# zju3dv/EnvGS

Hardware: AMD Instinct MI355X
Metric: train iters/s (fwd+bwd of the render hot path + Adam step, one 800x800 view per GPU per iter) + render Mpix/s (higher is better)
Workload: dtype f32

## Files before the change

envgs_amd/_lib.py:

```python
import ctypes
import os

import torch

HERE = os.path.dirname(os.path.abspath(__file__))
LIB_PATH = os.path.join(HERE, "libenvgs_hip.so")
_lib = None

c_void_p, c_int, c_uint32, c_size_t = ctypes.c_void_p, ctypes.c_int, ctypes.c_uint32, ctypes.c_size_t


class RasterCfg(ctypes.Structure):
    _fields_ = [("P", ctypes.c_int32), ("sh_degree", ctypes.c_int32), ("sh_coeffs", ctypes.c_int32),
                ("channels", ctypes.c_int32), ("width", ctypes.c_int32), ("height", ctypes.c_int32),
                ("bg_len", ctypes.c_int32), ("debug", ctypes.c_int32), ("scale_modifier", ctypes.c_float),
                ("tanfovx", ctypes.c_float), ("tanfovy", ctypes.c_float), ("feature_f16", ctypes.c_int32)]


class AdamTensor(ctypes.Structure):
    _fields_ = [("param", ctypes.c_void_p), ("grad", ctypes.c_void_p), ("exp_avg", ctypes.c_void_p), ("exp_avg_sq", ctypes.c_void_p),
                ("numel", ctypes.c_int64), ("lr", ctypes.c_float), ("step", ctypes.c_float)]


class RowsTensor(ctypes.Structure):
# ... 89 lines not shown
    "envgs_raster_sort_temp_bytes": (c_size_t, [c_uint32, ctypes.c_int32, ctypes.c_int32]),
    "envgs_raster_project": (c_int, [ctypes.POINTER(RasterCfg)] + [_P] * 15 + [_P, c_size_t, ctypes.POINTER(c_uint32), _P]),
    "envgs_raster_bin_and_render": (c_int, [ctypes.POINTER(RasterCfg), c_uint32] + [_P] * 7 + [_P, c_size_t] + [_P] * 7 + [_P]),
    "envgs_raster_render_audit": (c_int, [ctypes.POINTER(RasterCfg)] + [_P] * 11 + [ctypes.c_int32, _P, _P]),
    "envgs_raster_backward": (c_int, [ctypes.POINTER(RasterCfg), c_uint32] + [_P] * 29 + [_P]),
    "envgs_bvh_temp_bytes": (c_size_t, [ctypes.c_int32]),
    "envgs_bvh_node_floats": (c_size_t, [ctypes.c_int32]),
    "envgs_bvh_build": (c_int, [ctypes.c_int32, _P, _P, _P, _P, c_size_t, ctypes.c_int32, _P]),
    "envgs_bvh_refit": (c_int, [ctypes.c_int32, _P, _P, _P, _P, _P, c_size_t, ctypes.c_int32, _P]),
    "envgs_bvh_quality": (c_int, [ctypes.c_int32, _P, _P, _P]),
    "envgs_trace_ray_sort_temp_bytes": (c_size_t, [ctypes.c_int32]),
    "envgs_trace_ray_order": (c_int, [ctypes.c_int32, _P, _P, _P, ctypes.c_int32, _P, _P, _P, c_size_t, _P]),
    "envgs_trace_forward": (c_int, [ctypes.POINTER(TraceCfg)] + [_P] * 22 + [ctypes.POINTER(TraceLists), _P]),
    "envgs_trace_backward": (c_int, [ctypes.POINTER(TraceCfg)] + [_P] * 35 + [ctypes.POINTER(TraceLists), _P]),
    "envgs_trace_backward_join": (c_int, [_P]),
    "envgs_sh_colors_forward": (c_int, [ctypes.c_int32] * 4 + [_P] * 7 + [_P]),
    "envgs_sh_colors_backward": (c_int, [ctypes.c_int32] * 4 + [_P] * 9 + [_P]),
    "envgs_surfel_quads": (c_int, [ctypes.c_int32] + [_P] * 5 + [_P]),
    "envgs_blend_forward": (c_int, [ctypes.c_int32] * 3 + [_P] * 3 + [_P]),
    "envgs_blend_backward": (c_int, [ctypes.c_int32] * 3 + [_P] * 5 + [_P]),
    "envgs_bounce_rays_forward": (c_int, [ctypes.c_int32] + [_P] * 8 + [_P]),
    "envgs_bounce_rays_backward": (c_int, [ctypes.c_int32] + [_P] * 13 + [_P]),
    "envgs_bounce_blend_forward": (c_int, [ctypes.c_int32] + [_P] * 5 + [_P]),
    "envgs_bounce_blend_backward": (c_int, [ctypes.c_int32] + [_P] * 8 + [_P]),
    "envgs_bounce_pack_mid": (c_int, [ctypes.c_int32, _P, ctypes.c_int32, ctypes.c_int32] + [_P] * 8 + [_P]),
    "envgs_reflect_forward": (c_int, [ctypes.c_int32, ctypes.c_int32, ctypes.c_float] + [_P] * 8 + [_P]),
    "envgs_reflect_backward": (c_int, [ctypes.c_int32, ctypes.c_int32, ctypes.c_float] + [_P] * 11 + [_P]),
    "envgs_select_acc": (c_int, [ctypes.c_int32, ctypes.c_int32, ctypes.c_float, _P, _P, _P]),
    "envgs_reflect_filtered_forward": (c_int, [ctypes.c_int32, ctypes.c_int32, ctypes.c_float, ctypes.c_int32] + [_P] * 10 + [_P]),
    "envgs_reflect_filtered_backward": (c_int, [ctypes.c_int32, ctypes.c_int32, ctypes.c_float, ctypes.c_int32] + [_P] * 13 + [_P]),
# ... 95 lines not shown
```

envgs_amd/csrc/trace_api.hip:

```cpp
#include "trace_common.h"

#include <mutex>

namespace envgs {

constexpr int MAX_SEG = ENVGS_TRACE_MAX_SEG;

static int persistent_grid(int R, int per_cu = 8)
{
    int dev = 0, cus = 256;
    if (hipGetDevice(&dev) == hipSuccess) {
        int v = 0;
        if (hipDeviceGetAttribute(&v, hipDeviceAttributeMultiprocessorCount, dev) == hipSuccess && v > 0) cus = v;
    }
    const int want = (R + 63) / 64;
    const int cap = cus * per_cu;
    return want < cap ? (want > 0 ? want : 1) : cap;
}

static int stride_grid(int R, int per_block)
{
    const int want = (R + per_block - 1) / per_block;
    const int cap = 256 * 32;
    const int g = want < cap ? (want > 0 ? want : 1) : cap;
// ... 74 lines not shown
    return A;
}

static int bwd_order_classes()
{
    const int k = debug_switch(ENVGS_DBG_BALANCE) >> 8;
    return k > 0 ? k : ENVGS_BWD_ORDER_CLASSES;
}

static unsigned sparse_capacity(const envgs_trace_lists *L)
{
    return (unsigned)(L->sparse_cap > 0xFFFFFFF0ull ? 0xFFFFFFF0ull : L->sparse_cap);
}

static int forward_segment(const envgs_trace_cfg *cfg, const envgs_raster_cfg *dcfg, const envgs_trace_lists *L, const TraceArgs &S, hipStream_t st,
                           int seg_wgs, bool compact)
{
    const int rays_seg = (S.batch1 - S.batch0) * 64;
    {
        ProfScope p1(K_TRACE_COLLECT, st);
        const dim3 cg(persistent_grid(rays_seg, seg_wgs));
        const float4 *n4 = S.nodes + (size_t)(cfg->P > 1 ? cfg->P - 1 : 1) * 4;
        hipLaunchKernelGGL(collect_hits_coop, cg, dim3(256), 0, st, S, S.nodes, n4, S.srec);
    }
    ENVGS_CHECK_LAUNCH(dcfg, st);
    if (compact) {
        const int nb_seg = S.batch1 - S.batch0, nblk = (rays_seg + 255) / 256;
        unsigned *cntb = L->row_blk;
        const unsigned long long limit = (unsigned long long)L->compact_rows;
        unsigned *first_row = S.counter + ENVGS_CTR_SEG_FIRST_ROW + S.seg;
        hipLaunchKernelGGL(row_scan_blocks, dim3(1), dim3(256), 0, st, cntb + S.batch0, nb_seg, S.counter + ENVGS_CTR_ROW_CLAIM, first_row);
        hipLaunchKernelGGL(row_offsets, dim3(nblk), dim3(256), 0, st, S, cntb, L->row_off, (uint2 *)L->batch_rows, (const unsigned *)first_row, limit);
        ENVGS_CHECK_LAUNCH(dcfg, st);
    }
    {
        ProfScope p2(K_TRACE_SORT, st);
        const dim3 g(stride_grid(rays_seg, 4)), b(256);
        if (S.shp) hipLaunchKernelGGL((sort_composite_fwd<4, false, true>), g, b, 0, st, S);
        else hipLaunchKernelGGL((sort_composite_fwd<4, false, false>), g, b, 0, st, S);
        if (S.cap > 256) {
            const dim3 gl(min(stride_grid(rays_seg, 256), 512));
            if (S.cap <= 512) { if (S.shp) hipLaunchKernelGGL((sort_composite_fwd<8, true, true>), gl, b, 0, st, S); else hipLaunchKernelGGL((sort_composite_fwd<8, true, false>), gl, b, 0, st, S); }
            else { if (S.shp) hipLaunchKernelGGL((sort_composite_fwd<16, true, true>), gl, b, 0, st, S); else hipLaunchKernelGGL((sort_composite_fwd<16, true, false>), gl, b, 0, st, S); }
        }
    }
    ENVGS_CHECK_LAUNCH(dcfg, st);
    {
        ProfScope p8(K_TRACE_REGISTER, st);
        const dim3 gr(stride_grid(rays_seg, 64)), br(64 * RH_W);
// ... 63 lines not shown
    if (lists) {
        if (L->scan_temp_bytes < scan_temp_bytes(cfg->P * NCOPY)) return ENVGS_ERR_TEMP_TOO_SMALL;
        A.hits = (uint2 *)L->hit_lists; A.hit_cnt = L->hit_cnt; A.n_used = L->n_used; A.cap = L->cap;
        A.surf_cnt = L->surf_cnt; A.surf_off = L->surf_off; A.surf_acc = (unsigned long long *)L->surf_acc;
        const bool will_sort = L->ray_keys && L->ray_order && L->ray_sort_temp && !(A.exp & ENVGS_DBG_TRACE_NO_SORT);
        {
            int ib = 1;
            while ((1ll << ib) <= (long long)cfg->num_rays) ib++;
            A.wfrac = 40 - ib > 30 ? 30 : 40 - ib;
        }
        A.state = (float4 *)L->hit_state; A.entries = (unsigned long long *)L->entries; A.pairs = L->pairs; A.n_entries = L->n_entries;
        const bool compact = L->compact_rows > 0 && L->row_off && L->batch_rows && L->row_blk && L->hit_state;
        if (L->compact_rows > 0 && !compact) return ENVGS_ERR_BAD_ARG;
        A.state_plane = compact ? (size_t)L->compact_rows : (size_t)cfg->num_rays * (size_t)L->cap;
        A.colour_state = L->state_planes == 1 ? 1 : 0;
        if (compact) { A.row_off = L->row_off; A.batch_rows = (const uint2 *)L->batch_rows; A.batch_cnt = L->row_blk; }
        if (L->sparse_hits && L->sparse_cap > 0 && L->entries && L->pairs && L->hit_state) {
            const int sw = debug_switch(ENVGS_DBG_SPARSE);
            A.sparse = (uint4 *)L->sparse_hits;
            A.sparse_cap = sparse_capacity(L);
            A.sparse_max = sw > 0 ? (sw - 1 > 64 ? 64 : sw - 1) : 4;
        }
        if (L->sh_perm && shs && cfg->sh_coeffs == 16) {
            const size_t nw = (size_t)cfg->P * 48;
            FP.perm_blocks = (int)((nw + 255) / 256); FP.nb = (cfg->sh_degree + 1) * (cfg->sh_degree + 1); FP.f16 = cfg->feature_f16;
            FP.shs = (const void *)shs; FP.shp = L->sh_perm;
            A.shp = L->sh_perm;
        }
        const int nbatch_all = (cfg->num_rays + 63) / 64;
        int nseg = 2;
        if (debug_switch(ENVGS_DBG_SEGMENTS) > 0) nseg = debug_switch(ENVGS_DBG_SEGMENTS);
// ... 26 lines not shown
        }
        if (prepare_aside) { if (hipStreamWaitEvent(stream, ev_join[1], 0) != hipSuccess) return ENVGS_ERR_BAD_ARG; }
        else { const int rcp = launch_prepare(stream); if (rcp) return rcp; ENVGS_CHECK_LAUNCH(dcfg, stream); }
        if (nseg > 1) {
            if (hipEventRecord(ev_fork, stream) != hipSuccess) return ENVGS_ERR_BAD_ARG;
            for (int i = 1; i < nseg; i++)
                if (hipStreamWaitEvent(aux[i], ev_fork, 0) != hipSuccess) return ENVGS_ERR_BAD_ARG;
        }
        const int coop_wgs = (debug_switch(ENVGS_DBG_COLLECT_WGS) > 0 && debug_switch(ENVGS_DBG_COLLECT_WGS) <= 8) ? debug_switch(ENVGS_DBG_COLLECT_WGS)
                                                                                                                  : (nseg > 1 ? 4 : 8);
        for (int sg = 0; sg < nseg; sg++) {
            TraceArgs S = A;
            S.seg = sg;
            S.batch0 = (int)((long long)nbatch_all * sg / nseg);
            S.batch1 = (int)((long long)nbatch_all * (sg + 1) / nseg);
            const int rcs = forward_segment(cfg, dcfg, L, S, sg ? aux[sg] : stream, coop_wgs, compact); if (rcs) return rcs;
        }
        for (int i = 1; i < nseg; i++)
            if (hipEventRecord(ev_join[i], aux[i]) != hipSuccess || hipStreamWaitEvent(stream, ev_join[i], 0) != hipSuccess) return ENVGS_ERR_BAD_ARG;
        unsigned *bwd_order = (L->bwd_order && records_prepared(L)) ? L->bwd_order : nullptr;
        hipLaunchKernelGGL(unpack_surfel_acc, dim3((cfg->P + 255) / 256 + (bwd_order ? 1 : 0)), dim3(256), 0, stream, cfg->P, A.wfrac, A.surf_acc, L->surf_cnt, wet,
                           counters + ENVGS_CTR_RAY_FETCH, (const int *)L->n_entries, nbatch_all, bwd_order, bwd_order_classes());
        ENVGS_CHECK_LAUNCH(dcfg, stream);
        const int rc = launch_scan(L->surf_cnt, L->surf_off, cfg->P * NCOPY, L->scan_temp, L->scan_temp_bytes, stream); if (rc) return rc;
        A.only_overflow = 1;
    } else {
        const int rcp = launch_prepare(stream); if (rcp) return rcp;
        ENVGS_CHECK_LAUNCH(dcfg, stream);
    }
    { ProfScope p4(K_TRACE_KBUF_FWD, stream); hipLaunchKernelGGL(trace_fwd, dim3(persistent_grid(cfg->num_rays)), dim3(64), 0, stream, A, rh, rw); }
    ENVGS_CHECK_LAUNCH(dcfg, stream);
// ... 40 lines not shown
    if (A.exp & ENVGS_DBG_TRACE_RETIRED) return ENVGS_ERR_BAD_ARG;
    int rh, rw; ray_layout(cfg, &rh, &rw);
    bool deferred = false, have_records = false;
    int def_dev = 0;
    {
        ProfScope prof_(K_TRACE_BWD, stream);
        if (lists_wanted(cfg, L) && !lists_usable_bwd(cfg, L)) return ENVGS_ERR_BAD_ARG;
        if (lists_usable_bwd(cfg, L)) {
            A.hits = (uint2 *)L->hit_lists; A.hit_cnt = L->hit_cnt; A.n_used = L->n_used; A.cap = L->cap;
            if (L->ray_keys && L->ray_order && L->ray_sort_temp && !(A.exp & ENVGS_DBG_TRACE_NO_SORT)) A.order = L->ray_order + cfg->num_rays;
            if (L->records && L->num_records > 0 && records_prepared(L)) {
                A.surf_cnt = L->surf_cnt; A.surf_off = L->surf_off; A.records = L->records; A.num_records = L->num_records;
                A.state = (float4 *)L->hit_state; A.entries = (unsigned long long *)L->entries; A.pairs = L->pairs; A.n_entries = L->n_entries;
                if (L->compact_rows > 0) {
                    if (!L->row_off || !L->batch_rows) return ENVGS_ERR_BAD_ARG;
                    A.row_off = L->row_off; A.batch_rows = (const uint2 *)L->batch_rows;
                }
                A.state_plane = L->compact_rows > 0 ? (size_t)L->compact_rows : (size_t)cfg->num_rays * (size_t)L->cap;
                {
                    ProfScope p5(K_TRACE_LIST_BWD, stream);
                    const bool rgb_only = dL_drgb && !dL_ddpt && !dL_dacc && !dL_dnorm && !dL_daux;
                    if (L->state_planes == 1 && !rgb_only) return ENVGS_ERR_BAD_ARG;
                    const bool by_cost = L->bwd_order && !(debug_switch(ENVGS_DBG_BALANCE) & 1);
                    A.bwd_order = by_cost ? L->bwd_order : nullptr;
                    const dim3 g(by_cost ? (cfg->num_rays + 63) / 64 : stride_grid((cfg->num_rays + 63) / 64, 1));
                    if (rgb_only) hipLaunchKernelGGL((batch_surfel_bwd<true, false>), g, dim3(64), 0, stream, A);
                    else if (cfg->has_others) hipLaunchKernelGGL((batch_surfel_bwd<false, true>), g, dim3(64), 0, stream, A);
                    else hipLaunchKernelGGL((batch_surfel_bwd<false, false>), g, dim3(64), 0, stream, A);
                    if (L->sparse_hits && L->sparse_cap > 0) {
                        A.sparse = (uint4 *)L->sparse_hits;
                        A.sparse_cap = sparse_capacity(L);
// ... 47 lines not shown
```

envgs_amd/csrc/trace_collect.hip:

```cpp
#include "trace_common.h"

namespace envgs {

typedef float f32x2 __attribute__((ext_vector_type(2)));
constexpr int COOP_W = 4;
constexpr float COOP_REFRESH_OD = 1.0f;
constexpr int COOP_ODROW = 36;
constexpr int COOP_NBIN = 32;
constexpr int COOP_STK = 96;
constexpr int COOP_FRONT = 64;
constexpr int COOP_ITEMS = 256;
static_assert(COOP_ODROW % 4 == 0, "the bin rows are read with ds_read_b128");
constexpr float COOP_OD_SCALE = 65536.0f;
constexpr unsigned COOP_KILL_Q = (unsigned)(KILL_OD * 65536.0f);
struct CoopLds {
    unsigned od[64][COOP_ODROW];
    unsigned odtot[64];
    int cnt[64];
    unsigned long long items[2][COOP_ITEMS];
    int stk[COOP_W][COOP_STK];
    int nitems[2];
    int next, ovf, batch, pad;
};

__global__ void __launch_bounds__(256, 8)
collect_hits_coop(const TraceArgs A, const float4 *__restrict__ nodes, const float4 *__restrict__ nodes4, const float4 *__restrict__ srec)
{
    __shared__ CoopLds L;
#ifdef ENVGS_DIAG
// ... 60 lines not shown
            };
            const int ux = sign_of(dx, ix), uy = sign_of(dy, iy), uz = sign_of(dz, iz);
            if (vm != 0ull && ux < 2 && uy < 2 && uz < 2) oct = ux | (uy << 1) | (uz << 2);
        }
#endif

        unsigned long long c1 = c0;
        bool ovf = false;
        auto walk = [&]<int OCT>() {
        auto record_hit = [&](const SurfHit &h, const int sid) {
            const int slot = atomicAdd(&L.cnt[lane], 1);
            if (slot < A.cap) list[slot] = make_uint2(__float_as_uint(h.t), (unsigned)sid);
            const float x = (h.t - tA) * inv_bin_w;
            int b = x <= 0.0f ? 0 : (int)ceilf(x + 1e-3f);
            b = b > COOP_NBIN - 1 ? COOP_NBIN - 1 : b;
            const unsigned dep = (unsigned)(-__logf(1.0f - h.alpha) * COOP_OD_SCALE);
            atomicAdd(&L.od[lane][b], dep);
            atomicAdd(&L.odtot[lane], dep);
        };
        auto refresh_bound = [&]() {
            const unsigned tot = ENVGS_LDS_READ(L.odtot[lane]);
            if (__builtin_amdgcn_ballot_w64(tot >= COOP_KILL_Q && tot > seen + (unsigned)(COOP_REFRESH_OD * COOP_OD_SCALE)) != 0ull) {
                seen = tot;
                unsigned cum = 0u; int kb = COOP_NBIN - 1;
                const uint4 *row = reinterpret_cast<const uint4 *>(&L.od[lane][0]);
                asm volatile("" ::: "memory");
#pragma unroll
                for (int h = 0; h < COOP_NBIN / 16; h++) {
                    uint4 v[4];
#pragma unroll
                    for (int q = 0; q < 4; q++) v[q] = row[4 * h + q];
#pragma unroll
                    for (int q = 0; q < 4; q++) {
                        const unsigned e[4] = {v[q].x, v[q].y, v[q].z, v[q].w};
#pragma unroll
                        for (int j = 0; j < 4; j++) {
                            const int bin = 16 * h + 4 * q + j;
                            if (bin < COOP_NBIN - 1) { cum += e[j]; kb = (cum >= COOP_KILL_Q && kb == COOP_NBIN - 1) ? bin : kb; }
                        }
                    }
                }
                tkill = kb < COOP_NBIN - 1 ? tA + (float)kb * bin_w : tk_open;
            }
        };
        auto step = [&](const int cur_, unsigned long long (&kr)[4]) -> int {
            const int cur = __builtin_amdgcn_readfirstlane(cur_);
            const float4 *nd = nodes4 + (size_t)cur * 8;
            psteps++;
            float4 qa[4], qb[4];
#if defined(ENVGS_COOP_TIMING) && ENVGS_COOP_TIMING == 2
            const unsigned long long ta = __builtin_readcyclecounter();
            {
                typedef float f8_ __attribute__((ext_vector_type(8)));
                f8_ r0, r1, r2, r3;
                asm volatile("s_load_dwordx8 %0, %4, 0\n s_load_dwordx8 %1, %4, 32\n s_load_dwordx8 %2, %4, 64\n s_load_dwordx8 %3, %4, 96\n s_waitcnt lgkmcnt(0)"
// ... 157 lines not shown
        __syncthreads();
        const unsigned long long c3 = __builtin_readcyclecounter();
#if defined(ENVGS_COOP_TIMING) && ENVGS_COOP_TIMING == 3
        (void)c0; (void)c1; (void)c2; (void)c3;
#elif defined(ENVGS_COOP_TIMING)
        cyc_walk += c2 - c0; (void)c1; (void)c3;
#else
        cyc_expand += c1 - c0; cyc_walk += c2 - c1; cyc_wait += c3 - c2;
#endif
        if (wave == 0) {
            int n = L.cnt[lane];
            if (L.ovf) {
                n = A.cap + 1;
                if (lane == 0) atomicAdd(A.counter + ENVGS_CTR_STACK_OVERFLOWS, 1u);
            }
            if (valid) { A.hit_cnt[r] = n; found_tot += (unsigned)n; }
            int mx = n;
            for (int o = 32; o > 0; o >>= 1) mx = max(mx, __shfl_xor(mx, o));
            if (lane == 0) atomicMax((int *)(A.counter + ENVGS_CTR_MAX_LIST), mx);
            if (A.batch_cnt) {
                const float rows = wave_sum((valid && n <= A.cap) ? (float)n : 0.f);
                if (lane == 0) A.batch_cnt[A.batch0 + fb] = (unsigned)rows;
            }
        }
        __syncthreads();
    }
    if (A.stats) {
        const float ff = wave_sum((float)found_tot);
        if (lane == 0) {
            if (wave == 0) atomicAdd(A.stats + ENVGS_TOT_FOUND, (unsigned long long)ff);
            atomicAdd(A.stats + ENVGS_TOT_PACKET_NODES, (unsigned long long)psteps); atomicAdd(A.stats + ENVGS_TOT_PACKET_LEAVES, (unsigned long long)pleaves);
            atomicAdd(A.stats + ENVGS_TOT_COOP_EXPAND, cyc_expand); atomicAdd(A.stats + ENVGS_TOT_COOP_WALK, cyc_walk); atomicAdd(A.stats + ENVGS_TOT_COOP_WAIT, cyc_wait);
        }
    }
#undef ENVGS_LDS_READ
}

}
```

envgs_amd/csrc/trace_common.h:

```cpp
#ifndef ENVGS_TRACE_COMMON_H
#define ENVGS_TRACE_COMMON_H

#include "common.h"
#include "prof.h"
#include "sh_basis.h"

#include <cstdlib>
#include <cstring>

#include "../../include/envgs_trace.h"

namespace envgs {

constexpr int KBUF = 16;
constexpr int STACK = 64;
constexpr int NCOPY = 8;
constexpr int MAX_ROUNDS = 256;
constexpr float UV_MAX = 3.0f;
constexpr int MID = ENVGS_MID_CHANNELS;
constexpr int SREC = ENVGS_SREC_STRIDE;
constexpr int NODE = ENVGS_NODE_STRIDE;

struct SurfHit { float t, u, v, G, alpha, denom; bool ok; };

// ... 71 lines not shown
    int only_overflow;
    int batch0, batch1;
    uint4 *sparse;
    unsigned sparse_cap;
    int sparse_max;
    int reduce_adds;
    int seg;
    unsigned long long *entries;
    unsigned *pairs;
    int *n_entries;
    unsigned *long_list;
    float4 *state;
    size_t state_plane;
    int colour_state;
    unsigned *batch_cnt;
    const unsigned *row_off;
    const uint2 *batch_rows;
    const void *shp;
    const unsigned *bwd_order;
};

struct KBuf {
    float t[KBUF];
    int id[KBUF];
    int n;
    __device__ __forceinline__ void reset() {
#pragma unroll
        for (int i = 0; i < KBUF; i++) { t[i] = 3.0e38f; id[i] = 0x7fffffff; }
        n = 0;
    }
    __device__ __forceinline__ void insert(float ct, int cid) {
#pragma unroll
// ... 422 lines not shown
};
__global__ void __launch_bounds__(256) forward_prepare(const ForwardPrepare F);
__global__ void __launch_bounds__(64) trace_fwd(const TraceArgs A, const int ray_h, const int ray_w);
__global__ void __launch_bounds__(64) trace_bwd(const TraceArgs A, const int ray_h, const int ray_w);
__global__ void __launch_bounds__(256, 8)
collect_hits_coop(const TraceArgs A, const float4 *__restrict__ nodes, const float4 *__restrict__ nodes4, const float4 *__restrict__ srec);

template <int EMAX, bool LONG, bool QSH> __global__ void __launch_bounds__(256) sort_composite_fwd(const TraceArgs A);
extern template __global__ void __launch_bounds__(256) sort_composite_fwd<4, false, false>(const TraceArgs A);
extern template __global__ void __launch_bounds__(256) sort_composite_fwd<8, true, false>(const TraceArgs A);
extern template __global__ void __launch_bounds__(256) sort_composite_fwd<16, true, false>(const TraceArgs A);
extern template __global__ void __launch_bounds__(256) sort_composite_fwd<4, false, true>(const TraceArgs A);
extern template __global__ void __launch_bounds__(256) sort_composite_fwd<8, true, true>(const TraceArgs A);
extern template __global__ void __launch_bounds__(256) sort_composite_fwd<16, true, true>(const TraceArgs A);
template <bool CACHED> __global__ void __launch_bounds__(64 * RH_W) register_hits(const TraceArgs A);
__global__ void __launch_bounds__(256) row_scan_blocks(unsigned *__restrict__ blk, int n, unsigned *rows_used, unsigned *seg_base);
__global__ void __launch_bounds__(256) row_offsets(const TraceArgs A, const unsigned *__restrict__ blk, unsigned *__restrict__ row_off, uint2 *__restrict__ batch_rows,
                                                   const unsigned *__restrict__ seg_base, unsigned long long limit);
__global__ void __launch_bounds__(256) unpack_surfel_acc(int P, int wfrac, const unsigned long long *__restrict__ acc, unsigned *__restrict__ cnt,
                                                         float *__restrict__ wet, unsigned *ray_counter, const int *__restrict__ n_entries, int nbatch,
                                                         unsigned *__restrict__ bwd_order, int order_classes);
__global__ void __launch_bounds__(256) sparse_hits_bwd(const TraceArgs A, const int rgbo);
template <bool RGBO, bool OTH> __global__ void __attribute__((amdgpu_waves_per_eu(ENVGS_BSB_WAVES, ENVGS_BSB_WAVES))) __launch_bounds__(64) batch_surfel_bwd(const TraceArgs A);
extern template __global__ void __attribute__((amdgpu_waves_per_eu(ENVGS_BSB_WAVES, ENVGS_BSB_WAVES))) __launch_bounds__(64) batch_surfel_bwd<false, false>(const TraceArgs A);
extern template __global__ void __attribute__((amdgpu_waves_per_eu(ENVGS_BSB_WAVES, ENVGS_BSB_WAVES))) __launch_bounds__(64) batch_surfel_bwd<false, true>(const TraceArgs A);
extern template __global__ void __attribute__((amdgpu_waves_per_eu(ENVGS_BSB_WAVES, ENVGS_BSB_WAVES))) __launch_bounds__(64) batch_surfel_bwd<true, false>(const TraceArgs A);
__global__ void __launch_bounds__(256) reduce_surfel_records(const TraceArgs A);
__global__ void __launch_bounds__(256) finish_surfel_grads(int P, const float *__restrict__ rots, const float *__restrict__ geo_rec,
                                                           float *__restrict__ dmeans, float *__restrict__ dscales, float *__restrict__ dopac,
                                                           float *__restrict__ drots, float *__restrict__ dgrads3D);

}
#endif
// ... 1 lines not shown
```

envgs_amd/csrc/trace_lists.hip:

```cpp
#include "trace_common.h"

#ifndef ENVGS_SCF_KO
#define ENVGS_SCF_KO 0
#endif
namespace envgs {

template <int S>
__device__ __forceinline__ unsigned xlane(unsigned v)
{
    if constexpr (S == 1) return (unsigned)__builtin_amdgcn_update_dpp(0, (int)v, 0xB1, 0xf, 0xf, true);
    else if constexpr (S == 2) return (unsigned)__builtin_amdgcn_update_dpp(0, (int)v, 0x4E, 0xf, 0xf, true);
    else if constexpr (S == 32) {
        const envgs_u2 r = __builtin_amdgcn_permlane32_swap(v, v, false, false);
        return (threadIdx.x & 32) ? r.x : r.y;
    } else return (unsigned)__builtin_amdgcn_ds_swizzle((int)v, 0x1F | (S << 10));
}

template <int E, int SIZE, int STRIDE>
__device__ __forceinline__ void bitonic_layer(unsigned long long (&k)[E], const int lane)
{
    if constexpr (STRIDE >= 64) {
        constexpr int SE = STRIDE / 64;
#pragma unroll
        for (int e = 0; e < E; e++)
// ... 551 lines not shown
                    for (unsigned f = threadIdx.x; f < nfail; f += 64 * RH_W) {
                        const unsigned long long ev = ent[region - 1 - f];
                        const unsigned pv = prs[region - 1 - f];
                        A.sparse[fbase + f] = make_uint4((unsigned)base + (pv >> 16), pv & 0xFFFFu, (unsigned)(ev & 0xFFFFFFull), (unsigned)(ev >> 32));
                    }
                    if (threadIdx.x == 0) { if (A.n_entries) A.n_entries[2 * batch + 1] = 0; atomicSub(A.counter + ENVGS_CTR_BATCH_ENTRIES,nfail); }
                }
            }
        }
    }
}

template __global__ void register_hits<false>(const TraceArgs A);
template __global__ void register_hits<true>(const TraceArgs A);

__device__ __forceinline__ unsigned rows_of_slot(const TraceArgs &A, const int slot, const int slot_end)
{
    if (slot >= slot_end) return 0u;
    const int r = ray_of(A, slot);
    const int n = A.hit_cnt[r];
    return n > A.cap ? 0u : (unsigned)n;
}

__global__ void __launch_bounds__(256)
row_scan_blocks(unsigned *__restrict__ blk, int n, unsigned *rows_used, unsigned *seg_base)
{
    __shared__ unsigned wtot[4];
    __shared__ unsigned s_base;
    const int lane = threadIdx.x & 63, wave = threadIdx.x >> 6;
    if (threadIdx.x == 0) s_base = 0u;
    __syncthreads();
    constexpr int PRE = 8;
    unsigned pre[PRE][4];
#pragma unroll
    for (int c = 0; c < PRE; c++)
#pragma unroll
        for (int q = 0; q < 4; q++) { const int i = c * 1024 + 4 * (int)threadIdx.x + q; pre[c][q] = i < n ? blk[i] : 0u; }
    int c = 0;
    for (int c0 = 0; c0 < n; c0 += 1024, c++) {
        const int i0 = c0 + 4 * (int)threadIdx.x;
        unsigned v[4];
        if (c < PRE) {
#pragma unroll
            for (int q = 0; q < 4; q++) {
                v[q] = pre[0][q];
#pragma unroll
                for (int p_ = 1; p_ < PRE; p_++) v[q] = c == p_ ? pre[p_][q] : v[q];
            }
        } else {
#pragma unroll
            for (int q = 0; q < 4; q++) v[q] = i0 + q < n ? blk[i0 + q] : 0u;
        }
        const unsigned tsum = v[0] + v[1] + v[2] + v[3];
        unsigned x = tsum;
#pragma unroll
        for (int o = 1; o < 64; o <<= 1) { const unsigned y = (unsigned)__shfl_up((int)x, o); if (lane >= o) x += y; }
        if (lane == 63) wtot[wave] = x;
        __syncthreads();
        unsigned before = s_base;
        for (int w = 0; w < wave; w++) before += wtot[w];
        unsigned run = before + x - tsum;
#pragma unroll
        for (int q = 0; q < 4; q++) { if (i0 + q < n) blk[i0 + q] = run; run += v[q]; }
        __syncthreads();
        if (threadIdx.x == 255) s_base = before + x;
        __syncthreads();
    }
    if (threadIdx.x == 0 && rows_used && seg_base) *seg_base = atomicAdd(rows_used, s_base);
}

__global__ void __launch_bounds__(256)
row_offsets(const TraceArgs A, const unsigned *__restrict__ blk, unsigned *__restrict__ row_off, uint2 *__restrict__ batch_rows,
            const unsigned *__restrict__ seg_base, unsigned long long limit)
{
    const unsigned long long base = (unsigned long long)*seg_base;
    const int slot_end = min(A.R, A.batch1 * 64);
    const int slot = A.batch0 * 64 + (int)blockIdx.x * 256 + (int)threadIdx.x;
    const int lane = threadIdx.x & 63, batch = slot >> 6;
    if (batch >= A.batch1) return;
    const unsigned cnt = rows_of_slot(A, slot, slot_end);
    const float incl = wave_scan_add((float)cnt);
    const unsigned long long row0 = base + (unsigned long long)blk[batch];
    const unsigned long long row = row0 + (unsigned long long)((unsigned)incl - cnt);
    const bool fits = row + cnt <= limit;
    if (slot < slot_end) {
        row_off[slot] = (unsigned)(fits ? row : 0ull);
        if (!fits && cnt > 0u) {
            A.hit_cnt[ray_of(A, slot)] = A.cap + 1;
            atomicAdd(A.counter + ENVGS_CTR_RAYS_WITHOUT_ROWS, 1u);
        }
    }
    const unsigned tot = (unsigned)wave_bcast(incl, 63);
    if (lane == 0) {
        const unsigned long long end = row0 + tot < limit ? row0 + tot : limit;
        batch_rows[batch] = make_uint2((unsigned)(row0 < limit ? row0 : limit), (unsigned)(end > row0 ? end - row0 : 0ull));
    }
}

constexpr int ORDER_MAX_CLASSES = 1024;
constexpr int ORDER_SEGS = 4;
__device__ __forceinline__ int order_count(const int *__restrict__ n_entries, int b)
{
    const int c = n_entries[2 * b] + n_entries[2 * b + 1];
    return c < 0 ? 0 : (c > (1 << 20) ? (1 << 20) : c);
}
__device__ __forceinline__ int order_bin(int cnt, int maxc, int K)
{
    cnt = cnt > maxc ? maxc : cnt;
    return K - 1 - (int)(((unsigned)cnt * (unsigned)K) / ((unsigned)maxc + 1u));
}
__device__ void build_bwd_order(const int *__restrict__ n_entries, const int nbatch, unsigned *__restrict__ order, int K)
{
    __shared__ unsigned s_off[ORDER_MAX_CLASSES * ORDER_SEGS];
// ... 81 lines not shown
```

envgs_amd/tracing.py:

```python
from typing import NamedTuple

import torch
from torch import nn

from . import _lib


class SurfelTracingSettings(NamedTuple):
    image_height: int
    image_width: int
    tanfovx: float
    tanfovy: float
    bg: torch.Tensor
    scale_modifier: float
    viewmatrix: torch.Tensor
    projmatrix: torch.Tensor
    sh_degree: int
    campos: torch.Tensor
    prefiltered: bool
    debug: bool
    max_trace_depth: int
    specular_threshold: float


# ... 280 lines not shown
        if k.records and sparse:
            k.sparse_hits = _scratch((max(4096, rows if rows else R * cap), 4), torch.int32, dev)
            if SPARSE.get("poison") is not None:
                k.sparse_hits.fill_(int(SPARSE["poison"]))
            k.sparse_cap = k.sparse_hits.shape[0] if SPARSE.get("cap") is None else min(int(SPARSE["cap"]), k.sparse_hits.shape[0])
        lists = _trace_lists(k)
    p = _lib.ptr
    _lib.check(lib.envgs_trace_forward(cfg, p(nodes), p(ro), p(rd), p(means3D), p(scales), p(rotations), p(opacities), p(shs),
                                       p(colors_precomp), p(others_precomp), p(bg), p(srec), p(counters), p(rgb), p(dpt), p(acc),
                                       p(norm), p(dist), p(aux), p(mid), p(wet), p(final_T), lists, _stream(dev)), "envgs_trace_forward")
    records = k is not None and k.records
    LAST_STATS.update(P=P, R=R, caps=caps, rows=rows, counters=counters, n_entries=(k.n_entries if records else None), cap=cap,
                      lists=((k.hit_lists, k.n_used, k.hit_cnt) if (cap and KEEP_LISTS["on"]) else None),
                      records=(dict(sparse_hits=k.sparse_hits, sparse_cap=k.sparse_cap, entries=k.entries, pairs=k.pairs,
                                    n_entries=k.n_entries, batch_rows=(k.batch_rows.view(-1, 2) if rows else None),
                                    ray_order=(k.ray_order[R:] if k.ray_order is not None else None), surf_cnt=k.surf_cnt, surf_off=k.surf_off,
                                    bwd_order=k.bwd_order)
                               if (records and KEEP_LISTS["on"]) else None))
    if cap:
        if records and not KEEP_LISTS["on"]:
            k.hit_lists = lists.hit_lists = None
        caps.publish(counters, dev, rays=R)
        if records:
            k.n_rec_host, k.n_rec_claim = caps.pinned_word()
            k.n_rec_host.copy_(k.surf_off.view(-1)[NCOPY * P - 1:NCOPY * P], non_blocking=True)
            k.n_rec_event = torch.cuda.Event(); k.n_rec_event.record(torch.cuda.current_stream(dev))
    saved = _Saved(cfg=cfg, nodes=nodes, ro=ro, rd=rd, means3D=means3D, scales=scales, rotations=rotations, opacities=opacities,
                   shs=shs, colors_precomp=colors_precomp, others=others_precomp, bg=bg, srec=srec, counters=counters,
                   rgb=(rgb if ND == 1 else mid[:, 13:16].contiguous()),
                   dpt=dpt, acc=acc, norm=norm, aux=aux, final_T=final_T, lead=lead, lists=lists, keep=k, cap=cap)
# ... 400 lines not shown
```

include/envgs_trace.h:

```cpp
#ifndef ENVGS_TRACE_H
#define ENVGS_TRACE_H

#include <stddef.h>
#include <stdint.h>

#include "envgs_raster.h"

#ifdef __cplusplus
extern "C" {
#endif

#define ENVGS_NODE_STRIDE 16
#define ENVGS_SREC_STRIDE 16
#define ENVGS_GEOREC_STRIDE 16
#define ENVGS_MID_CHANNELS 16
#define ENVGS_WIDE_EMPTY ((int32_t)0x80000000)

typedef struct envgs_trace_cfg {
    int32_t P;
    int32_t num_rays;
    int32_t sh_degree;
    int32_t sh_coeffs;
    int32_t max_trace_depth;
    int32_t start_from_first;
// ... 104 lines not shown
                                   const float *ray_o, const float *ray_d,
                                   const float *means3D, const float *scales, const float *rotations, const float *opacities,
                                   const float *shs, const float *colors_precomp, const float *others_precomp, const float *bg,
                                   const float *srec, uint32_t *counters,
                                   const float *rgb, const float *dpt, const float *acc, const float *norm, const float *aux,
                                   const float *final_T,
                                   const float *dL_drgb, const float *dL_ddpt, const float *dL_dacc, const float *dL_dnorm,
                                   const float *dL_daux,
                                   float *geo_rec,
                                   float *dmeans3D, float *dgrads3D, float *dscales, float *drots, float *dopacities,
                                   float *dshs, float *dcolors, float *dothers, float *dray_o, float *dray_d,
                                   const envgs_trace_lists *lists, void *stream);

ENVGS_API int envgs_trace_backward_join(void *stream);

#ifdef __cplusplus
}
#endif
#endif
```

Baseline: 144.6.

## Fuse compact row allocation into collect kernel and cheapen kill-bin depth math

```diff
diff --git a/envgs_amd/_lib.py b/envgs_amd/_lib.py
--- a/envgs_amd/_lib.py
+++ b/envgs_amd/_lib.py
@@ -127,6 +127,7 @@
     "envgs_trace_forward": (c_int, [ctypes.POINTER(TraceCfg)] + [_P] * 22 + [ctypes.POINTER(TraceLists), _P]),
     "envgs_trace_backward": (c_int, [ctypes.POINTER(TraceCfg)] + [_P] * 35 + [ctypes.POINTER(TraceLists), _P]),
     "envgs_trace_backward_join": (c_int, [_P]),
+    "envgs_trace_bound_selftest": (c_int, [_P, _P, ctypes.c_int32, _P, _P, _P]),
     "envgs_sh_colors_forward": (c_int, [ctypes.c_int32] * 4 + [_P] * 7 + [_P]),
     "envgs_sh_colors_backward": (c_int, [ctypes.c_int32] * 4 + [_P] * 9 + [_P]),
     "envgs_surfel_quads": (c_int, [ctypes.c_int32] + [_P] * 5 + [_P]),
diff --git a/envgs_amd/csrc/collect_bound.h b/envgs_amd/csrc/collect_bound.h
--- /dev/null
+++ b/envgs_amd/csrc/collect_bound.h
@@ -0,0 +1,29 @@
+#pragma once
+#include "trace_common.h"
+
+namespace envgs {
+
+constexpr int COOP_NBIN = 32;
+constexpr float COOP_OD_SCALE = 65536.0f;
+constexpr unsigned COOP_KILL_Q = (unsigned)(KILL_OD * 65536.0f);
+
+constexpr float COOP_OD_MARGIN = 1.0f;
+__device__ __forceinline__ unsigned coop_od_units(const float alpha)
+{
+    const float l2 = __builtin_amdgcn_logf(1.0f - alpha);
+    const float u = __builtin_fmaf(l2, -0.693147180559945f * COOP_OD_SCALE, -COOP_OD_MARGIN);
+    return (unsigned)fmaxf(u, 0.0f);
+}
+
+__device__ __forceinline__ void coop_kill_bin16(const uint4 (&v)[4], const int h, unsigned &cum, int &kb)
+{
+#pragma unroll
+    for (int q = 0; q < 4; q++) {
+        const unsigned e[4] = {v[q].x, v[q].y, v[q].z, v[q].w};
+#pragma unroll
+        for (int j = 0; j < 4; j++)
+            if (16 * h + 4 * q + j < COOP_NBIN - 1) { cum += e[j]; kb += cum < COOP_KILL_Q ? 1 : 0; }
+    }
+}
+
+}
diff --git a/envgs_amd/csrc/trace_api.hip b/envgs_amd/csrc/trace_api.hip
--- a/envgs_amd/csrc/trace_api.hip
+++ b/envgs_amd/csrc/trace_api.hip
@@ -112,7 +112,7 @@
 }
 
 static int forward_segment(const envgs_trace_cfg *cfg, const envgs_raster_cfg *dcfg, const envgs_trace_lists *L, const TraceArgs &S, hipStream_t st,
-                           int seg_wgs, bool compact)
+                           int seg_wgs)
 {
     const int rays_seg = (S.batch1 - S.batch0) * 64;
     {
@@ -122,15 +122,6 @@
         hipLaunchKernelGGL(collect_hits_coop, cg, dim3(256), 0, st, S, S.nodes, n4, S.srec);
     }
     ENVGS_CHECK_LAUNCH(dcfg, st);
-    if (compact) {
-        const int nb_seg = S.batch1 - S.batch0, nblk = (rays_seg + 255) / 256;
-        unsigned *cntb = L->row_blk;
-        const unsigned long long limit = (unsigned long long)L->compact_rows;
-        unsigned *first_row = S.counter + ENVGS_CTR_SEG_FIRST_ROW + S.seg;
-        hipLaunchKernelGGL(row_scan_blocks, dim3(1), dim3(256), 0, st, cntb + S.batch0, nb_seg, S.counter + ENVGS_CTR_ROW_CLAIM, first_row);
-        hipLaunchKernelGGL(row_offsets, dim3(nblk), dim3(256), 0, st, S, cntb, L->row_off, (uint2 *)L->batch_rows, (const unsigned *)first_row, limit);
-        ENVGS_CHECK_LAUNCH(dcfg, st);
-    }
     {
         ProfScope p2(K_TRACE_SORT, st);
         const dim3 g(stride_grid(rays_seg, 4)), b(256);
@@ -224,7 +215,7 @@
         if (L->compact_rows > 0 && !compact) return ENVGS_ERR_BAD_ARG;
         A.state_plane = compact ? (size_t)L->compact_rows : (size_t)cfg->num_rays * (size_t)L->cap;
         A.colour_state = L->state_planes == 1 ? 1 : 0;
-        if (compact) { A.row_off = L->row_off; A.batch_rows = (const uint2 *)L->batch_rows; A.batch_cnt = L->row_blk; }
+        if (compact) { A.row_off = L->row_off; A.batch_rows = (uint2 *)L->batch_rows; A.batch_cnt = L->row_blk; }
         if (L->sparse_hits && L->sparse_cap > 0 && L->entries && L->pairs && L->hit_state) {
             const int sw = debug_switch(ENVGS_DBG_SPARSE);
             A.sparse = (uint4 *)L->sparse_hits;
@@ -281,7 +272,7 @@
             S.seg = sg;
             S.batch0 = (int)((long long)nbatch_all * sg / nseg);
             S.batch1 = (int)((long long)nbatch_all * (sg + 1) / nseg);
-            const int rcs = forward_segment(cfg, dcfg, L, S, sg ? aux[sg] : stream, coop_wgs, compact); if (rcs) return rcs;
+            const int rcs = forward_segment(cfg, dcfg, L, S, sg ? aux[sg] : stream, coop_wgs); if (rcs) return rcs;
         }
         for (int i = 1; i < nseg; i++)
             if (hipEventRecord(ev_join[i], aux[i]) != hipSuccess || hipStreamWaitEvent(stream, ev_join[i], 0) != hipSuccess) return ENVGS_ERR_BAD_ARG;
@@ -352,7 +343,7 @@
                 A.state = (float4 *)L->hit_state; A.entries = (unsigned long long *)L->entries; A.pairs = L->pairs; A.n_entries = L->n_entries;
                 if (L->compact_rows > 0) {
                     if (!L->row_off || !L->batch_rows) return ENVGS_ERR_BAD_ARG;
-                    A.row_off = L->row_off; A.batch_rows = (const uint2 *)L->batch_rows;
+                    A.row_off = L->row_off; A.batch_rows = (uint2 *)L->batch_rows;
                 }
                 A.state_plane = L->compact_rows > 0 ? (size_t)L->compact_rows : (size_t)cfg->num_rays * (size_t)L->cap;
                 {
diff --git a/envgs_amd/csrc/trace_collect.hip b/envgs_amd/csrc/trace_collect.hip
--- a/envgs_amd/csrc/trace_collect.hip
+++ b/envgs_amd/csrc/trace_collect.hip
@@ -1,4 +1,5 @@
 #include "trace_common.h"
+#include "collect_bound.h"
 
 namespace envgs {
 
@@ -6,13 +7,10 @@
 constexpr int COOP_W = 4;
 constexpr float COOP_REFRESH_OD = 1.0f;
 constexpr int COOP_ODROW = 36;
-constexpr int COOP_NBIN = 32;
 constexpr int COOP_STK = 96;
 constexpr int COOP_FRONT = 64;
 constexpr int COOP_ITEMS = 256;
 static_assert(COOP_ODROW % 4 == 0, "the bin rows are read with ds_read_b128");
-constexpr float COOP_OD_SCALE = 65536.0f;
-constexpr unsigned COOP_KILL_Q = (unsigned)(KILL_OD * 65536.0f);
 struct CoopLds {
     unsigned od[64][COOP_ODROW];
     unsigned odtot[64];
@@ -103,7 +101,7 @@
             const float x = (h.t - tA) * inv_bin_w;
             int b = x <= 0.0f ? 0 : (int)ceilf(x + 1e-3f);
             b = b > COOP_NBIN - 1 ? COOP_NBIN - 1 : b;
-            const unsigned dep = (unsigned)(-__logf(1.0f - h.alpha) * COOP_OD_SCALE);
+            const unsigned dep = coop_od_units(h.alpha);
             atomicAdd(&L.od[lane][b], dep);
             atomicAdd(&L.odtot[lane], dep);
         };
@@ -111,7 +109,7 @@
             const unsigned tot = ENVGS_LDS_READ(L.odtot[lane]);
             if (__builtin_amdgcn_ballot_w64(tot >= COOP_KILL_Q && tot > seen + (unsigned)(COOP_REFRESH_OD * COOP_OD_SCALE)) != 0ull) {
                 seen = tot;
-                unsigned cum = 0u; int kb = COOP_NBIN - 1;
+                unsigned cum = 0u; int kb = 0;
                 const uint4 *row = reinterpret_cast<const uint4 *>(&L.od[lane][0]);
                 asm volatile("" ::: "memory");
 #pragma unroll
@@ -119,15 +117,7 @@
                     uint4 v[4];
 #pragma unroll
                     for (int q = 0; q < 4; q++) v[q] = row[4 * h + q];
-#pragma unroll
-                    for (int q = 0; q < 4; q++) {
-                        const unsigned e[4] = {v[q].x, v[q].y, v[q].z, v[q].w};
-#pragma unroll
-                        for (int j = 0; j < 4; j++) {
-                            const int bin = 16 * h + 4 * q + j;
-                            if (bin < COOP_NBIN - 1) { cum += e[j]; kb = (cum >= COOP_KILL_Q && kb == COOP_NBIN - 1) ? bin : kb; }
-                        }
-                    }
+                    coop_kill_bin16(v, h, cum, kb);
                 }
                 tkill = kb < COOP_NBIN - 1 ? tA + (float)kb * bin_w : tk_open;
             }
@@ -315,14 +305,33 @@
                 n = A.cap + 1;
                 if (lane == 0) atomicAdd(A.counter + ENVGS_CTR_STACK_OVERFLOWS, 1u);
             }
-            if (valid) { A.hit_cnt[r] = n; found_tot += (unsigned)n; }
+            if (valid) found_tot += (unsigned)n;
             int mx = n;
             for (int o = 32; o > 0; o >>= 1) mx = max(mx, __shfl_xor(mx, o));
             if (lane == 0) atomicMax((int *)(A.counter + ENVGS_CTR_MAX_LIST), mx);
-            if (A.batch_cnt) {
-                const float rows = wave_sum((valid && n <= A.cap) ? (float)n : 0.f);
-                if (lane == 0) A.batch_cnt[A.batch0 + fb] = (unsigned)rows;
-            }
+            if (A.batch_cnt && A.row_off && A.batch_rows) {
+                const unsigned cnt = (valid && n <= A.cap) ? (unsigned)n : 0u;
+                const unsigned incl = wave_scan_add_u32(cnt);
+                const unsigned tot = (unsigned)__builtin_amdgcn_readlane((int)incl, 63);
+                unsigned first = 0u;
+                if (lane == 0) { first = atomicAdd(A.counter + ENVGS_CTR_ROW_CLAIM, tot); A.batch_cnt[A.batch0 + fb] = tot; }
+                const unsigned long long limit = (unsigned long long)A.state_plane;
+                const unsigned long long row0 = (unsigned long long)(unsigned)__builtin_amdgcn_readfirstlane((int)first);
+                const unsigned long long row = row0 + (unsigned long long)(incl - cnt);
+                const bool fits = row + cnt <= limit;
+                if (valid) {
+                    A.row_off[base + lane] = (unsigned)(fits ? row : 0ull);
+                    if (!fits && cnt > 0u) {
+                        n = A.cap + 1;
+                        atomicAdd(A.counter + ENVGS_CTR_RAYS_WITHOUT_ROWS, 1u);
+                    }
+                }
+                if (lane == 0) {
+                    const unsigned long long end = row0 + tot < limit ? row0 + tot : limit;
+                    A.batch_rows[A.batch0 + fb] = make_uint2((unsigned)(row0 < limit ? row0 : limit), (unsigned)(end > row0 ? end - row0 : 0ull));
+                }
+            }
+            if (valid) A.hit_cnt[r] = n;
         }
         __syncthreads();
     }
@@ -337,4 +346,52 @@
 #undef ENVGS_LDS_READ
 }
 
-}
+__global__ void __launch_bounds__(256)
+bound_selftest_units(const unsigned lo, const unsigned hi, unsigned long long *__restrict__ res)
+{
+    unsigned long long over = 0ull, shortfall = 0ull, swept = 0ull;
+    for (unsigned long long b = (unsigned long long)lo + (unsigned long long)blockIdx.x * 256ull + threadIdx.x; b <= (unsigned long long)hi;
+         b += (unsigned long long)gridDim.x * 256ull) {
+        const float alpha = __uint_as_float((unsigned)b);
+        const long long exact = (long long)floor(-log1p(-(double)alpha) * 65536.0), got = (long long)coop_od_units(alpha);
+        over += got > exact ? 1ull : 0ull;
+        shortfall = exact - got > (long long)shortfall ? (unsigned long long)(exact - got) : shortfall;
+        swept++;
+    }
+    if (over) atomicAdd(&res[0], over);
+    atomicMax(&res[1], shortfall);
+    atomicAdd(&res[2], swept);
+}
+__global__ void __launch_bounds__(256)
+bound_selftest_bins(const unsigned *__restrict__ rows, const int n, unsigned *__restrict__ kb_new, unsigned *__restrict__ kb_old)
+{
+    const int i = (int)(blockIdx.x * 256u + threadIdx.x);
+    if (i >= n) return;
+    const uint4 *row = reinterpret_cast<const uint4 *>(rows + (size_t)i * COOP_NBIN);
+    unsigned cum = 0u; int kb = 0;
+    for (int h = 0; h < COOP_NBIN / 16; h++) {
+        uint4 v[4];
+        for (int q = 0; q < 4; q++) v[q] = row[4 * h + q];
+        coop_kill_bin16(v, h, cum, kb);
+    }
+    kb_new[i] = (unsigned)kb;
+    unsigned c2 = 0u; int k2 = COOP_NBIN - 1;
+    for (int bin = 0; bin < COOP_NBIN - 1; bin++) { c2 += rows[(size_t)i * COOP_NBIN + bin]; k2 = (c2 >= COOP_KILL_Q && k2 == COOP_NBIN - 1) ? bin : k2; }
+    kb_old[i] = (unsigned)k2;
+}
+
+}
+
+extern "C" int envgs_trace_bound_selftest(uint64_t *res3, const uint32_t *bin_rows, int32_t n_rows, uint32_t *kb_new, uint32_t *kb_old, void *stream_)
+{
+    using namespace envgs;
+    if (!res3 || n_rows < 0 || (n_rows > 0 && (!bin_rows || !kb_new || !kb_old))) return ENVGS_ERR_BAD_ARG;
+    hipStream_t st = (hipStream_t)stream_;
+    if (hipMemsetAsync(res3, 0, 3 * sizeof(uint64_t), st) != hipSuccess) return ENVGS_ERR_BAD_ARG;
+    const float lo = ALPHA_MIN, hi = ALPHA_CAP;
+    hipLaunchKernelGGL(bound_selftest_units, dim3(4096), dim3(256), 0, st, __builtin_bit_cast(unsigned, lo), __builtin_bit_cast(unsigned, hi),
+                       (unsigned long long *)res3);
+    if (n_rows > 0)
+        hipLaunchKernelGGL(bound_selftest_bins, dim3((unsigned)((n_rows + 255) / 256)), dim3(256), 0, st, bin_rows, (int)n_rows, kb_new, kb_old);
+    return (int)hipGetLastError();
+}
diff --git a/envgs_amd/csrc/trace_common.h b/envgs_amd/csrc/trace_common.h
--- a/envgs_amd/csrc/trace_common.h
+++ b/envgs_amd/csrc/trace_common.h
@@ -109,8 +109,8 @@
     size_t state_plane;
     int colour_state;
     unsigned *batch_cnt;
-    const unsigned *row_off;
-    const uint2 *batch_rows;
+    unsigned *row_off;
+    uint2 *batch_rows;
     const void *shp;
     const unsigned *bwd_order;
 };
@@ -563,9 +563,6 @@
 extern template __global__ void __launch_bounds__(256) sort_composite_fwd<8, true, true>(const TraceArgs A);
 extern template __global__ void __launch_bounds__(256) sort_composite_fwd<16, true, true>(const TraceArgs A);
 template <bool CACHED> __global__ void __launch_bounds__(64 * RH_W) register_hits(const TraceArgs A);
-__global__ void __launch_bounds__(256) row_scan_blocks(unsigned *__restrict__ blk, int n, unsigned *rows_used, unsigned *seg_base);
-__global__ void __launch_bounds__(256) row_offsets(const TraceArgs A, const unsigned *__restrict__ blk, unsigned *__restrict__ row_off, uint2 *__restrict__ batch_rows,
-                                                   const unsigned *__restrict__ seg_base, unsigned long long limit);
 __global__ void __launch_bounds__(256) unpack_surfel_acc(int P, int wfrac, const unsigned long long *__restrict__ acc, unsigned *__restrict__ cnt,
                                                          float *__restrict__ wet, unsigned *ray_counter, const int *__restrict__ n_entries, int nbatch,
                                                          unsigned *__restrict__ bwd_order, int order_classes);
diff --git a/envgs_amd/csrc/trace_lists.hip b/envgs_amd/csrc/trace_lists.hip
--- a/envgs_amd/csrc/trace_lists.hip
+++ b/envgs_amd/csrc/trace_lists.hip
@@ -589,89 +589,6 @@
 template __global__ void register_hits<false>(const TraceArgs A);
 template __global__ void register_hits<true>(const TraceArgs A);
 
-__device__ __forceinline__ unsigned rows_of_slot(const TraceArgs &A, const int slot, const int slot_end)
-{
-    if (slot >= slot_end) return 0u;
-    const int r = ray_of(A, slot);
-    const int n = A.hit_cnt[r];
-    return n > A.cap ? 0u : (unsigned)n;
-}
-
-__global__ void __launch_bounds__(256)
-row_scan_blocks(unsigned *__restrict__ blk, int n, unsigned *rows_used, unsigned *seg_base)
-{
-    __shared__ unsigned wtot[4];
-    __shared__ unsigned s_base;
-    const int lane = threadIdx.x & 63, wave = threadIdx.x >> 6;
-    if (threadIdx.x == 0) s_base = 0u;
-    __syncthreads();
-    constexpr int PRE = 8;
-    unsigned pre[PRE][4];
-#pragma unroll
-    for (int c = 0; c < PRE; c++)
-#pragma unroll
-        for (int q = 0; q < 4; q++) { const int i = c * 1024 + 4 * (int)threadIdx.x + q; pre[c][q] = i < n ? blk[i] : 0u; }
-    int c = 0;
-    for (int c0 = 0; c0 < n; c0 += 1024, c++) {
-        const int i0 = c0 + 4 * (int)threadIdx.x;
-        unsigned v[4];
-        if (c < PRE) {
-#pragma unroll
-            for (int q = 0; q < 4; q++) {
-                v[q] = pre[0][q];
-#pragma unroll
-                for (int p_ = 1; p_ < PRE; p_++) v[q] = c == p_ ? pre[p_][q] : v[q];
-            }
-        } else {
-#pragma unroll
-            for (int q = 0; q < 4; q++) v[q] = i0 + q < n ? blk[i0 + q] : 0u;
-        }
-        const unsigned tsum = v[0] + v[1] + v[2] + v[3];
-        unsigned x = tsum;
-#pragma unroll
-        for (int o = 1; o < 64; o <<= 1) { const unsigned y = (unsigned)__shfl_up((int)x, o); if (lane >= o) x += y; }
-        if (lane == 63) wtot[wave] = x;
-        __syncthreads();
-        unsigned before = s_base;
-        for (int w = 0; w < wave; w++) before += wtot[w];
-        unsigned run = before + x - tsum;
-#pragma unroll
-        for (int q = 0; q < 4; q++) { if (i0 + q < n) blk[i0 + q] = run; run += v[q]; }
-        __syncthreads();
-        if (threadIdx.x == 255) s_base = before + x;
-        __syncthreads();
-    }
-    if (threadIdx.x == 0 && rows_used && seg_base) *seg_base = atomicAdd(rows_used, s_base);
-}
-
-__global__ void __launch_bounds__(256)
-row_offsets(const TraceArgs A, const unsigned *__restrict__ blk, unsigned *__restrict__ row_off, uint2 *__restrict__ batch_rows,
-            const unsigned *__restrict__ seg_base, unsigned long long limit)
-{
-    const unsigned long long base = (unsigned long long)*seg_base;
-    const int slot_end = min(A.R, A.batch1 * 64);
-    const int slot = A.batch0 * 64 + (int)blockIdx.x * 256 + (int)threadIdx.x;
-    const int lane = threadIdx.x & 63, batch = slot >> 6;
-    if (batch >= A.batch1) return;
-    const unsigned cnt = rows_of_slot(A, slot, slot_end);
-    const float incl = wave_scan_add((float)cnt);
-    const unsigned long long row0 = base + (unsigned long long)blk[batch];
-    const unsigned long long row = row0 + (unsigned long long)((unsigned)incl - cnt);
-    const bool fits = row + cnt <= limit;
-    if (slot < slot_end) {
-        row_off[slot] = (unsigned)(fits ? row : 0ull);
-        if (!fits && cnt > 0u) {
-            A.hit_cnt[ray_of(A, slot)] = A.cap + 1;
-            atomicAdd(A.counter + ENVGS_CTR_RAYS_WITHOUT_ROWS, 1u);
-        }
-    }
-    const unsigned tot = (unsigned)wave_bcast(incl, 63);
-    if (lane == 0) {
-        const unsigned long long end = row0 + tot < limit ? row0 + tot : limit;
-        batch_rows[batch] = make_uint2((unsigned)(row0 < limit ? row0 : limit), (unsigned)(end > row0 ? end - row0 : 0ull));
-    }
-}
-
 constexpr int ORDER_MAX_CLASSES = 1024;
 constexpr int ORDER_SEGS = 4;
 __device__ __forceinline__ int order_count(const int *__restrict__ n_entries, int b)
diff --git a/envgs_amd/tracing.py b/envgs_amd/tracing.py
--- a/envgs_amd/tracing.py
+++ b/envgs_amd/tracing.py
@@ -318,6 +318,7 @@
                       lists=((k.hit_lists, k.n_used, k.hit_cnt) if (cap and KEEP_LISTS["on"]) else None),
                       records=(dict(sparse_hits=k.sparse_hits, sparse_cap=k.sparse_cap, entries=k.entries, pairs=k.pairs,
                                     n_entries=k.n_entries, batch_rows=(k.batch_rows.view(-1, 2) if rows else None),
+                                    row_off=(k.row_off if rows else None), row_blk=(k.row_blk[:nbatch] if rows else None),
                                     ray_order=(k.ray_order[R:] if k.ray_order is not None else None), surf_cnt=k.surf_cnt, surf_off=k.surf_off,
                                     bwd_order=k.bwd_order)
                                if (records and KEEP_LISTS["on"]) else None))
diff --git a/include/envgs_trace.h b/include/envgs_trace.h
--- a/include/envgs_trace.h
+++ b/include/envgs_trace.h
@@ -142,6 +142,8 @@
 
 ENVGS_API int envgs_trace_backward_join(void *stream);
 
+ENVGS_API int envgs_trace_bound_selftest(uint64_t *res3, const uint32_t *bin_rows, int32_t n_rows, uint32_t *kb_new, uint32_t *kb_old, void *stream);
+
 #ifdef __cplusplus
 }
 #endif
```

New measurement: 145.5 (median of 3 runs). No clear change (+0.6%).
